# waabox/domain-mcp-server

Hardware: AMD Instinct MI355X
Metric: classes indexed/sec (higher is better)
Workload: dtype n/a (CPU text indexing); 1 GPU; model=synthetic-java-spring-monorepo-2000-classes, global_batch=2000, parallelism=dp1 (one repo per rank), enrichment=none

## Files before the change

native/srcscan/project.cpp:

```cpp
#include <algorithm>
#include <chrono>
#include <dirent.h>
#include <string>
#include <unordered_map>
#include <unordered_set>

#include "srcscan.hpp"

namespace srcscan {

void go_project_files(const std::string& root, int threads, std::string& module, std::vector<FileRec>& files,
                      std::string* go_json);

namespace {

struct Entry {
    std::string name;
    bool is_dir;
};

std::vector<Entry> entries(const std::string& dir) {
    std::vector<std::pair<std::string, bool>> raw;
    std::vector<Entry> out;
    if (!list_dir(dir, raw)) return out;
// ... 41 lines not shown
    w.str_array("deps", f.deps);
    w.key("params");
    w.begin_obj();
    for (auto& kv : f.params) w.str_array(kv.first, kv.second);
    w.end_obj();
    w.key("methods");
    w.begin_arr();
    for (auto& m : f.methods) {
        w.begin_obj();
        w.kv("name", m.name);
        w.kv_int("line", m.line);
        w.kv_opt("httpMethod", m.has_http_method ? &m.http_method : nullptr);
        w.kv_opt("httpPath", m.has_http_path ? &m.http_path : nullptr);
        w.str_array("exceptions", m.exceptions);
        w.end_obj();
    }
    w.end_arr();
    w.end_obj();
}

void scan_java(const std::string& root, const ScanOptions& opt, ScanResult& res) {
    std::vector<FileRec>& files = res.files;
    const std::string src_root = "src/main/java";
    std::string abs_src = join_path(root, src_root);
    if (!dir_exists(abs_src)) return;
    std::vector<std::string> rels;
    auto t = std::chrono::steady_clock::now();
    walk(abs_src, "", [](const std::string& n) { return ends_with(n, ".java"); },
         [](const std::string&) { return false; }, rels);
    res.walk_us = us_since(t);
    t = std::chrono::steady_clock::now();
    files.resize(rels.size());
    std::vector<std::string> sources(rels.size());
    parallel_for(rels.size(), opt.threads, [&](size_t k) {
        FileRec& f = files[k];
        f.rel_path = src_root + "/" + rels[k];
        f.abs_path = join_path(root, f.rel_path);
        f.identifier = dotted(strip_ext(rels[k], ".java"));
        std::string src;
        if (!read_file(f.abs_path, src)) return;
        analyze_java(src, f);
    });
    for (auto& f : files) if (!f.parsed) ++res.skipped;
    res.analyze_us = us_since(t);
    t = std::chrono::steady_clock::now();
    std::unordered_set<std::string> known;
    known.reserve(files.size() * 2);
    for (auto& f : files) known.insert(f.identifier);
    parallel_for(files.size(), opt.threads, [&](size_t k) {
        FileRec& f = files[k];
        std::unordered_set<std::string> seen;
        std::unordered_map<std::string, std::string> import_map;
        for (auto& imp : f.imports) {
            if (imp.is_asterisk) continue;
            std::string fq = imp.imported;
            if (imp.is_static) {
                size_t d = fq.rfind('.');
                fq = (d != std::string::npos && d > 0) ? fq.substr(0, d) : std::string();
            }
            if (fq.empty()) continue;
            size_t d = fq.rfind('.');
            if (d != std::string::npos && d > 0) import_map[fq.substr(d + 1)] = fq;
            if (known.count(fq) && seen.insert(fq).second) f.deps.push_back(fq);
        }
        for (auto& m : f.methods) {
            if (!m.params_eligible || m.param_types.empty()) continue;
            std::vector<std::string> matched;
            for (auto& ty : m.param_types) {
                if (ty.empty()) continue;
                if (known.count(ty)) { matched.push_back(ty); continue; }
                auto it = import_map.find(ty);
                if (it != import_map.end() && known.count(it->second)) { matched.push_back(it->second); continue; }
                if (!f.package_name.empty()) {
                    std::string same = f.package_name + "." + ty;
                    if (known.count(same)) matched.push_back(same);
                }
            }
            if (matched.empty()) continue;
            bool replaced = false;
            for (auto& kv : f.params)
                if (kv.first == m.name) { kv.second = matched; replaced = true; break; }
            if (!replaced) f.params.emplace_back(m.name, matched);
        }
    });
    res.resolve_us = us_since(t);
}

const std::unordered_set<std::string> kTsExcludedDirs = {"node_modules", "dist", ".next", "build",
                                                         "coverage", "__tests__", "__mocks__"};

bool ts_source_file(const std::string& name) {
    if (!(ends_with(name, ".ts") || ends_with(name, ".tsx") || ends_with(name, ".js") || ends_with(name, ".jsx")))
        return false;
    if (contains(name, ".spec.") || contains(name, ".test.")) return false;
    if (ends_with(name, ".d.ts")) return false;
    return true;
}

void scan_ts(const std::string& root, const ScanOptions& opt, std::vector<FileRec>& files, int& skipped,
             FrameworkInfo& fw, std::string& source_root) {
    std::string pkg;
    if (!read_file(join_path(root, "package.json"), pkg)) pkg = "{}";
    fw = detect_framework(pkg);
    if (!opt.framework.empty()) fw.name = opt.framework;
    source_root = dir_exists(join_path(root, fw.source_root)) ? fw.source_root : "src";
    std::string abs_src = join_path(root, source_root);
    std::vector<std::string> rels;
    if (dir_exists(abs_src))
        walk(abs_src, "", ts_source_file, [](const std::string& n) { return kTsExcludedDirs.count(n) > 0; }, rels);
    files.resize(rels.size());
    std::string fw_name = fw.name;
    parallel_for(rels.size(), opt.threads, [&](size_t k) {
        FileRec& f = files[k];
        f.rel_path = source_root + "/" + rels[k];
        f.abs_path = join_path(root, f.rel_path);
        std::string r = rels[k];
        size_t dot = r.rfind('.');
        size_t slash = r.rfind('/');
        if (dot != std::string::npos && dot > 0 && (slash == std::string::npos || dot > slash + 1 || dot > slash))
            r = r.substr(0, dot);
        f.identifier = dotted(r);
        std::string src;
        if (!read_file(f.abs_path, src, opt.max_file_bytes)) return;
        bool jsx = !ends_with(f.rel_path, ".ts");
        analyze_ts(src, f.rel_path, fw_name, jsx, f);
    });
    std::vector<FileRec> kept;
    kept.reserve(files.size());
    for (auto& f : files) {
        if (f.parsed) kept.push_back(std::move(f));
        else ++skipped;
    }
    files.swap(kept);
    std::unordered_set<std::string> known;
    for (auto& f : files) known.insert(f.identifier);
    const std::string abs_root_norm = normalize_path(abs_src);
    auto resolve = [&](const std::string& import_path, const std::string& file_rel) -> std::string {
        std::string dir = file_rel;
        size_t s = dir.rfind('/');
        dir = s == std::string::npos ? std::string() : dir.substr(0, s);
        std::string full = normalize_path(join_path(join_path(root, dir), import_path));
        std::string prefix = abs_root_norm + "/";
        if (!starts_with(full, prefix)) return std::string();
        std::string cand = dotted(full.substr(prefix.size()));
        if (known.count(cand)) return cand;
        std::string idx = cand + ".index";
        if (known.count(idx)) return idx;
        return std::string();
    };
    parallel_for(files.size(), opt.threads, [&](size_t k) {
        FileRec& f = files[k];
        std::unordered_set<std::string> seen;
        std::unordered_map<std::string, std::string> type_map;
        for (auto& imp : f.imports) {
            if (!starts_with(imp.source, ".")) continue;
            std::string r = resolve(imp.source, f.rel_path);
            if (r.empty()) continue;
            if (seen.insert(r).second) f.deps.push_back(r);
            type_map[imp.local] = r;
        }
        for (auto& m : f.methods) {
            std::vector<std::string> matched;
            for (auto& ty : m.param_types) {
                auto it = type_map.find(ty);
                if (it != type_map.end() && known.count(it->second)) matched.push_back(it->second);
            }
            if (matched.empty()) continue;
            bool replaced = false;
            for (auto& kv : f.params)
                if (kv.first == m.name) { kv.second = matched; replaced = true; break; }
            if (!replaced) f.params.emplace_back(m.name, matched);
        }
    });
}

}

std::string detect_language(const std::string& root) {
    if (file_exists(join_path(root, "go.mod"))) return "go";
    if (file_exists(join_path(root, "package.json")) && !file_exists(join_path(root, "pom.xml")) &&
        !file_exists(join_path(root, "build.gradle")) && !file_exists(join_path(root, "build.gradle.kts")))
        return "typescript";
    return "java";
}

ScanResult scan_project(const std::string& root, const ScanOptions& opt) {
    ScanResult r;
    scan_project_into(root, opt, r);
    return r;
}

void scan_project_into(const std::string& root, const ScanOptions& opt, ScanResult& r) {
    auto t0 = std::chrono::steady_clock::now();
    std::string lang = opt.language;
    if (lang == "auto" || lang.empty()) lang = detect_language(root);
    if (lang == "ts" || lang == "js" || lang == "javascript" || lang == "node") lang = "typescript";
    if (lang == "typescript") {
        scan_ts(root, opt, r.files, r.skipped, r.framework, r.source_root);
        r.has_framework = true;
    } else if (lang == "go") {
        go_project_files(root, opt.threads, r.module, r.files, opt.go_doc ? &r.go_json : nullptr);
    } else {
        lang = "java";
        r.source_root = "src/main/java";
        scan_java(root, opt, r);
    }
    r.language = lang;
    r.elapsed_us = std::chrono::duration_cast<std::chrono::microseconds>(std::chrono::steady_clock::now() - t0).count();
}

std::string scan_result_json(const ScanResult& r) {
    JsonWriter w;
    w.begin_obj();
    w.kv("language", r.language);
    w.kv("sourceRoot", r.source_root);
    w.key("framework");
    if (r.has_framework) {
        w.begin_obj();
        w.kv("name", r.framework.name);
        w.kv("sourceRoot", r.framework.source_root);
        w.key("features");
        w.begin_obj();
        for (auto& kv : r.framework.features) w.kv(kv.first, kv.second);
        w.end_obj();
        w.end_obj();
    } else {
        w.value_null();
    }
    if (r.language == "go") w.kv("module", r.module);
    w.key("stats");
    w.begin_obj();
// ... 93 lines not shown
```

native/srcscan/pymodule.cpp:

```cpp
#include <pybind11/pybind11.h>
#include <pybind11/stl.h>
#include <sys/random.h>

#include <cctype>
#include <chrono>
#include <cstring>
#include <deque>
#include <memory>
#include <thread>
#include <unordered_map>
#include <vector>

#include "bulkwriter.hpp"
#include "gitobj.hpp"
#include "graphjson.hpp"
#include "srcscan.hpp"
#include "wire.hpp"

namespace py = pybind11;

namespace {

dbw::Batch to_batch(const std::string& sql, py::handle rows) {
    dbw::Batch b;
    b.sql = sql;
    PyObject* seq = PySequence_Fast(rows.ptr(), "rows must be a sequence");
    if (!seq) throw py::error_already_set();
    py::object keep = py::reinterpret_steal<py::object>(seq);
    const Py_ssize_t n = PySequence_Fast_GET_SIZE(seq);
    if (n == 0) return b;
    PyObject** items = PySequence_Fast_ITEMS(seq);
    PyObject* first = items[0];
    if (!PyTuple_Check(first)) throw py::type_error("rows must be tuples");
    b.ncols = static_cast<int>(PyTuple_GET_SIZE(first));
    b.values.resize(static_cast<size_t>(n) * b.ncols);
    for (Py_ssize_t r = 0; r < n; ++r) {
        PyObject* row = items[r];
        if (!PyTuple_Check(row) || PyTuple_GET_SIZE(row) != b.ncols) throw py::type_error("ragged rows");
        for (int c = 0; c < b.ncols; ++c) {
            PyObject* o = PyTuple_GET_ITEM(row, c);
            dbw::Value& v = b.values[static_cast<size_t>(r) * b.ncols + c];
            if (o == Py_None) {
                v.kind = dbw::Value::Null;
            } else if (PyUnicode_Check(o)) {
                Py_ssize_t len = 0;
                const char* s = PyUnicode_AsUTF8AndSize(o, &len);
                if (!s) throw py::error_already_set();
                v.kind = dbw::Value::Text;
                v.p = s;
                v.n = static_cast<int32_t>(len);
            } else if (PyBool_Check(o) || PyLong_Check(o)) {
                v.kind = dbw::Value::Int;
                v.i = PyLong_AsLongLong(o);
                if (v.i == -1 && PyErr_Occurred()) throw py::error_already_set();
            } else if (PyFloat_Check(o)) {
                v.kind = dbw::Value::Real;
                v.d = PyFloat_AS_DOUBLE(o);
            } else {
                throw py::type_error("unsupported column value type");
            }
        }
    }
    return b;
}

srcscan::ScanResult scan_mounted(py::list files, const std::string& language, int threads,
                                 const std::string& framework, bool go_doc = true) {
    const auto t = std::chrono::steady_clock::now();
    std::vector<py::object> hold;
    hold.reserve(files.size());
    std::vector<std::pair<std::string, std::string_view>> tree;
    tree.reserve(files.size());
    for (auto item : files) {
        auto tup = item.cast<py::tuple>();
        if (tup.size() != 2) throw py::type_error("files: (path, bytes) pairs expected");
        PyObject* content = tup[1].ptr();
        char* data = nullptr;
        Py_ssize_t n = 0;
        if (!PyBytes_Check(content) || PyBytes_AsStringAndSize(content, &data, &n) < 0)
            throw py::type_error("files: content must be bytes");
        tree.emplace_back(tup[0].cast<std::string>(), std::string_view(data, static_cast<size_t>(n)));
        hold.push_back(std::move(tup));
    }
    py::gil_scoped_release release;
    std::string root = srcscan::vfs_mount_views(tree);
    const long long mount_us =
        std::chrono::duration_cast<std::chrono::microseconds>(std::chrono::steady_clock::now() - t).count();
    srcscan::ScanOptions opt;
    opt.language = language;
    opt.threads = threads;
    opt.framework = framework;
    opt.go_doc = go_doc;
    try {
        srcscan::ScanResult r = srcscan::scan_project(root, opt);
        r.mount_us = mount_us;
        srcscan::vfs_unmount(root);
        return r;
    } catch (...) {
        srcscan::vfs_unmount(root);
        throw;
    }
}

py::str pystr(const std::string& s) {
    PyObject* o = PyUnicode_DecodeUTF8(s.data(), static_cast<Py_ssize_t>(s.size()), "replace");
    if (!o) throw py::error_already_set();
    return py::reinterpret_steal<py::str>(o);
}

void json_str_list_ascii(PyObject* seq, std::string& out) {
    static const char* hex = "0123456789abcdef";
    out.push_back('[');
    const Py_ssize_t n = PySequence_Fast_GET_SIZE(seq);
    PyObject** items = PySequence_Fast_ITEMS(seq);
    for (Py_ssize_t i = 0; i < n; ++i) {
        if (i) out.append(", ");
        PyObject* o = items[i];
        if (!PyUnicode_Check(o)) throw py::type_error("exception names must be str");
        out.push_back('"');
        const Py_ssize_t len = PyUnicode_GET_LENGTH(o);
        const int kind = PyUnicode_KIND(o);
        const void* data = PyUnicode_DATA(o);
        for (Py_ssize_t k = 0; k < len; ++k) {
            const Py_UCS4 c = PyUnicode_READ(kind, data, k);
            auto u4 = [&](unsigned v) {
                out.append("\\u");
                for (int sh = 12; sh >= 0; sh -= 4) out.push_back(hex[(v >> sh) & 15]);
            };
            switch (c) {
                case '"': out.append("\\\""); break;
                case '\\': out.append("\\\\"); break;
                case '\n': out.append("\\n"); break;
                case '\r': out.append("\\r"); break;
                case '\t': out.append("\\t"); break;
// ... 156 lines not shown
        PyObject* methods = PyList_New(static_cast<Py_ssize_t>(f.methods.size()));
        if (!methods) throw py::error_already_set();
        for (size_t i = 0; i < f.methods.size(); ++i) {
            const srcscan::MethodRec& m = f.methods[i];
            PyObject* exc = PyTuple_New(static_cast<Py_ssize_t>(m.exceptions.size()));
            if (!exc) throw py::error_already_set();
            for (size_t j = 0; j < m.exceptions.size(); ++j) PyTuple_SET_ITEM(exc, j, shared.get(m.exceptions[j]));
            PyObject* obj = mtype->tp_alloc(mtype, 5);
            if (!obj) throw py::error_already_set();
            PyTuple_SET_ITEM(obj, 0, fresh(m.name));
            PyTuple_SET_ITEM(obj, 1, PyLong_FromLong(m.line));
            PyTuple_SET_ITEM(obj, 2, m.has_http_method ? shared.get(m.http_method) : Py_NewRef(Py_None));
            PyTuple_SET_ITEM(obj, 3, m.has_http_path ? fresh(m.http_path) : Py_NewRef(Py_None));
            PyTuple_SET_ITEM(obj, 4, exc);
            PyList_SET_ITEM(methods, i, obj);
        }
        PyObject* rec = PyTuple_New(8);
        if (!rec) throw py::error_already_set();
        PyTuple_SET_ITEM(rec, 0, fresh(f.rel_path));
        PyTuple_SET_ITEM(rec, 1, fresh(f.identifier));
        PyTuple_SET_ITEM(rec, 2, shared.get(f.class_type));
        PyTuple_SET_ITEM(rec, 3, PyBool_FromLong(f.entry_point));
        PyTuple_SET_ITEM(rec, 4, shared.get(f.package_name));
        PyTuple_SET_ITEM(rec, 5, shared_list(f.deps));
        PyTuple_SET_ITEM(rec, 6, params);
        PyTuple_SET_ITEM(rec, 7, methods);
        PyList_SET_ITEM(files.ptr(), k, rec);
    }
    d["files"] = files;
    d["go"] = r.go_json.empty() ? py::object(py::none()) : py::object(pystr(r.go_json));
    return d;
}

struct Uuid7Gen {
    unsigned long long ms = 0, hi = 0, lo = 0;
    Uuid7Gen() {
        unsigned char seed[10];
        if (getrandom(seed, sizeof(seed), 0) != (ssize_t)sizeof(seed)) throw std::runtime_error("getrandom failed");
        ms = (unsigned long long)std::chrono::duration_cast<std::chrono::milliseconds>(
                 std::chrono::system_clock::now().time_since_epoch())
                 .count();
        hi = ((unsigned long long)(seed[0] & 0x07) << 8) | seed[1];
        for (int j = 2; j < 10; ++j) lo = (lo << 8) | seed[j];
        lo &= 0x1FFFFFFFFFFFFFFFull;
    }
    void next(char* s) {
        static const char* hex = "0123456789abcdef";
        unsigned char b[16];
        for (int j = 0; j < 6; ++j) b[j] = (unsigned char)(ms >> (8 * (5 - j)));
        b[6] = (unsigned char)(0x70 | ((hi >> 8) & 0x0F));
        b[7] = (unsigned char)(hi & 0xFF);
        b[8] = (unsigned char)(0x80 | ((lo >> 56) & 0x3F));
        for (int j = 9; j < 16; ++j) b[j] = (unsigned char)(lo >> (8 * (15 - j)));
        if (++lo >> 62) {
            lo = 0;
            ++hi;
        }
        int k = 0;
        for (int j = 0; j < 16; ++j) {
            if (j == 4 || j == 6 || j == 8 || j == 10) s[k++] = '-';
            s[k++] = hex[b[j] >> 4];
            s[k++] = hex[b[j] & 15];
        }
    }
};

void json_ascii_list(const std::vector<std::string>& v, std::string& out) {
    static const char* hex = "0123456789abcdef";
    auto u4 = [&](unsigned c) {
        out += "\\u";
        for (int sh = 12; sh >= 0; sh -= 4) out += hex[(c >> sh) & 15];
    };
    out = "[";
    for (size_t i = 0; i < v.size(); ++i) {
        if (i) out += ", ";
        out += '"';
        const std::string& s = v[i];
        for (size_t k = 0; k < s.size();) {
            unsigned char c = (unsigned char)s[k];
            unsigned cp = c;
            size_t len = 1;
            if (c >= 0xF0 && k + 3 < s.size() + 0) { cp = ((c & 7u) << 18) | ((s[k + 1] & 63u) << 12) | ((s[k + 2] & 63u) << 6) | (s[k + 3] & 63u); len = 4; }
            else if (c >= 0xE0 && k + 2 < s.size()) { cp = ((c & 15u) << 12) | ((s[k + 1] & 63u) << 6) | (s[k + 2] & 63u); len = 3; }
            else if (c >= 0xC0 && k + 1 < s.size()) { cp = ((c & 31u) << 6) | (s[k + 1] & 63u); len = 2; }
            k += len;
            if (cp == '"') out += "\\\"";
            else if (cp == '\\') out += "\\\\";
            else if (cp == '\n') out += "\\n";
            else if (cp == '\r') out += "\\r";
            else if (cp == '\t') out += "\\t";
            else if (cp == '\b') out += "\\b";
            else if (cp == '\f') out += "\\f";
            else if (cp < 0x20 || (cp >= 0x7f && cp < 0x10000)) u4(cp);
            else if (cp >= 0x10000) {
                cp -= 0x10000;
                u4(0xD800 + (cp >> 10));
                u4(0xDC00 + (cp & 0x3FF));
            } else out += (char)cp;
        }
        out += '"';
    }
    out += "]";
}

struct StaticRowsSpec {
    dbw::BulkWriter* writer = nullptr;
    std::string pid, now, commit, cls_sql, meth_sql;
    bool commit_null = false;
};

struct StaticRowsKeep {
    std::shared_ptr<const srcscan::ScanResult> r;
    StaticRowsSpec spec;
    std::string ids;
    std::vector<size_t> first;
    std::deque<std::string> strings;
};

const std::string& normalize_class_type(const std::string& t) {
    static const std::string kTypes[] = {"CONTROLLER", "SERVICE", "REPOSITORY", "ENTITY", "DTO",
                                         "CONFIGURATION", "LISTENER", "UTILITY", "EXCEPTION", "OTHER"};
    for (const std::string& k : kTypes) {
        if (k.size() != t.size()) continue;
        bool eq = true;
        for (size_t i = 0; i < t.size() && eq; ++i) eq = std::toupper((unsigned char)t[i]) == k[i];
        if (eq) return k;
    }
    return kTypes[9];
}

void emit_static_rows(const std::shared_ptr<StaticRowsKeep>& keep) {
    const srcscan::ScanResult& r = *keep->r;
    const StaticRowsSpec& spec = keep->spec;
    std::unordered_map<std::string_view, size_t> last;
    last.reserve(r.files.size() * 2);
    size_t n_ids = 0;
    for (size_t k = 0; k < r.files.size(); ++k) last[r.files[k].identifier] = k;
    for (size_t k = 0; k < r.files.size(); ++k)
        if (last[r.files[k].identifier] == k) n_ids += 1 + r.files[k].methods.size();
    keep->ids.resize(36 * n_ids);
    keep->first.assign(r.files.size(), std::string::npos);
    Uuid7Gen gen;
    size_t at = 0;
    const int chunk = 256;
    RowBuilder cls(spec.cls_sql, 10), meth(spec.meth_sql, 10);
    int pending = 0;
    auto flush = [&]() {
        cls.b.keep = keep;
        meth.b.keep = keep;
        if (!cls.empty()) spec.writer->put(std::move(cls.b));
        if (!meth.empty()) spec.writer->put(std::move(meth.b));
        cls = RowBuilder(spec.cls_sql, 10);
        meth = RowBuilder(spec.meth_sql, 10);
        pending = 0;
    };
    auto sv = [](RowBuilder& b, const std::string& s) { b.text(s.data(), (Py_ssize_t)s.size()); };
    for (size_t k = 0; k < r.files.size(); ++k) {
        const srcscan::FileRec& f = r.files[k];
        if (last[f.identifier] != k) continue;
        if (pending == chunk) flush();
        ++pending;
        keep->first[k] = at;
        const char* cid = &keep->ids[at];
        gen.next(&keep->ids[at]);
        at += 36;
        const std::string& ident = f.identifier;
        const size_t dot = ident.rfind('.');
        cls.text(cid, 36);
        sv(cls, spec.pid);
        sv(cls, ident);
        if (dot != std::string::npos) cls.text(ident.data() + dot + 1, (Py_ssize_t)(ident.size() - dot - 1));
        else sv(cls, ident);
        if (dot != std::string::npos) cls.text(ident.data(), (Py_ssize_t)dot); else cls.null();
        sv(cls, normalize_class_type(f.class_type));
        cls.null();
        sv(cls, f.rel_path);
        sv(cls, spec.now);
        if (spec.commit_null) cls.null(); else sv(cls, spec.commit);
        for (const srcscan::MethodRec& m : f.methods) {
            gen.next(&keep->ids[at]);
            meth.text(&keep->ids[at], 36);
            at += 36;
            meth.text(cid, 36);
            sv(meth, m.name);
            meth.null();
            meth.text("[]", 2);
            if (m.exceptions.empty()) {
                meth.text("[]", 2);
            } else {
                keep->strings.emplace_back();
                json_ascii_list(m.exceptions, keep->strings.back());
                sv(meth, keep->strings.back());
            }
            if (m.has_http_method) sv(meth, m.http_method); else meth.null();
            if (m.has_http_path) sv(meth, m.http_path); else meth.null();
            meth.integer(m.line);
            sv(meth, spec.now);
        }
    }
    flush();
}

py::tuple phase1_rows(dbw::BulkWriter& writer, py::list order, py::dict units, py::object ids, py::str pid,
                      py::str now, py::handle commit_hash, const std::string& cls_sql, const std::string& meth_sql,
                      const std::string& param_sql, py::handle method_info_cls, int chunk, py::object graph_targets,
                      py::object pre_ids) {
    if (!PyType_Check(method_info_cls.ptr()) ||
        !PyType_IsSubtype((PyTypeObject*)method_info_cls.ptr(), &PyTuple_Type))
        throw py::type_error("method_info_cls must be a tuple subclass");
    auto* mi_type = (PyTypeObject*)method_info_cls.ptr();
    const bool given = !ids.is_none();
    if (given && !PyList_Check(ids.ptr())) throw py::type_error("ids must be a list or None");
    const bool pre = !pre_ids.is_none();
    if (pre && (given || !PyDict_Check(pre_ids.ptr()))) throw py::type_error("pre_ids must be a dict (and ids None)");
    const Py_ssize_t n_ids = given ? PyList_GET_SIZE(ids.ptr()) : 0;
    Py_ssize_t next_id = 0;
    py::list generated;
    Uuid7Gen gen;
    auto nid = [&]() -> PyObject* {
        if (given) {
            if (next_id >= n_ids) throw py::value_error("phase1_rows: ran out of ids");
            return PyList_GET_ITEM(ids.ptr(), next_id++);
        }
        char buf[36];
        gen.next(buf);
        PyObject* o = PyUnicode_FromStringAndSize(buf, 36);
        if (!o || PyList_Append(generated.ptr(), o) < 0) {
            Py_XDECREF(o);
            throw py::error_already_set();
        }
        Py_DECREF(o);
// ... 221 lines not shown
                py::object posn = py::int_(p);
                PyObject* f = PyTuple_Pack(2, posn.ptr(), t);
                if (!f) throw py::error_already_set();
                py::object keep_f = py::reinterpret_steal<py::object>(f);
                py::object link = py::reinterpret_steal<py::object>(make_record(mpl_type, f));
                lks.append(link);
            }
            if (lks.empty()) continue;
            if (!gper) {
                gper = PyDict_GetItemWithError(g_mparams.ptr(), key);
                if (!gper) {
                    if (PyErr_Occurred()) throw py::error_already_set();
                    py::dict fresh;
                    if (PyDict_SetItem(g_mparams.ptr(), key, fresh.ptr()) < 0) throw py::error_already_set();
                    gper = fresh.ptr();
                }
            }
            PyObject* lst = PyDict_GetItemWithError(gper, mname);
            if (!lst) {
                if (PyErr_Occurred()) throw py::error_already_set();
                if (PyDict_SetItem(gper, mname, lks.ptr()) < 0) throw py::error_already_set();
            } else if (PyList_SetSlice(lst, PY_SSIZE_T_MAX, PY_SSIZE_T_MAX, lks.ptr()) < 0) {
                throw py::error_already_set();
            }
        }
    }
    if (!par.empty()) writer.put(std::move(par.b));
    return py::make_tuple(n_cls, n_meth, n_par, class_ids, class_types, method_infos, methods_by_ident, links,
                          generated);
}

}

py::dict objects_and_rows(std::shared_ptr<const srcscan::ScanResult> shared, py::handle method_cls, py::object rows) {
    std::shared_ptr<StaticRowsKeep> keep;
    std::thread emitter;
    std::atomic<long long> emit_us{0};
    if (!rows.is_none() && shared->language != "go") {
        py::tuple rt = rows.cast<py::tuple>();
        if (rt.size() != 6) throw py::value_error("rows must have 6 items");
        keep = std::make_shared<StaticRowsKeep>();
        keep->r = shared;
        StaticRowsSpec& spec = keep->spec;
        spec.writer = &rt[0].cast<dbw::BulkWriter&>();
        spec.pid = rt[1].cast<std::string>();
        spec.now = rt[2].cast<std::string>();
        spec.commit_null = rt[3].is_none();
        if (!spec.commit_null) spec.commit = rt[3].cast<std::string>();
        spec.cls_sql = rt[4].cast<std::string>();
        spec.meth_sql = rt[5].cast<std::string>();
        emitter = std::thread([keep, &emit_us] {
            const auto t = std::chrono::steady_clock::now();
            emit_static_rows(keep);
            emit_us = std::chrono::duration_cast<std::chrono::microseconds>(
                          std::chrono::steady_clock::now() - t).count();
        });
    }
    py::dict d;
    try {
        const auto t = std::chrono::steady_clock::now();
        d = scan_result_objects(*shared, method_cls);
        py::dict(d["stats"])["phaseUs"].cast<py::dict>()["objects"] =
            std::chrono::duration_cast<std::chrono::microseconds>(std::chrono::steady_clock::now() - t)
                .count();
    } catch (...) {
        if (emitter.joinable()) {
            py::gil_scoped_release release;
            emitter.join();
        }
        throw;
    }
    if (emitter.joinable()) {
        {
            py::gil_scoped_release release;
            emitter.join();
        }
        py::dict(d["stats"])["phaseUs"].cast<py::dict>()["rows"] = emit_us.load();
        py::dict row_ids;
        for (size_t k = 0; k < shared->files.size(); ++k) {
            const size_t at = keep->first[k];
            if (at == std::string::npos) continue;
            const size_t nm = shared->files[k].methods.size();
            py::list mids(nm);
            for (size_t j = 0; j < nm; ++j) mids[j] = py::str(&keep->ids[at + 36 * (j + 1)], 36);
            row_ids[pystr(shared->files[k].identifier)] = py::make_tuple(py::str(&keep->ids[at], 36), mids);
        }
        d["rowIds"] = row_ids;
    }
    keep.reset();
    std::thread([](std::shared_ptr<const srcscan::ScanResult>) {}, std::move(shared)).detach();
    return d;
}

PYBIND11_MODULE(_srcscan, m) {
    m.doc() = "Native Java / TypeScript / Go source front-ends for dmcp";
    m.def(
        "scan_project",
        [](const std::string& root, const std::string& language, int threads, const std::string& framework) {
            std::string out;
            {
                py::gil_scoped_release release;
                srcscan::ScanOptions opt;
                opt.language = language;
                opt.threads = threads;
                opt.framework = framework;
                out = srcscan::scan_project_json(root, opt);
            }
            return py::bytes(out);
        },
        py::arg("root"), py::arg("language") = "auto", py::arg("threads") = 0, py::arg("framework") = "");
    m.def(
        "scan_sources",
        [](py::list files, const std::string& language, int threads, const std::string& framework) {
            std::vector<std::pair<std::string, std::string>> tree;
            tree.reserve(files.size());
            for (auto item : files) {
                auto tup = item.cast<py::tuple>();
                tree.emplace_back(tup[0].cast<std::string>(), tup[1].cast<std::string>());
            }
            std::string out;
            {
                py::gil_scoped_release release;
                std::string root = srcscan::vfs_mount(std::move(tree));
                srcscan::ScanOptions opt;
                opt.language = language;
                opt.threads = threads;
                opt.framework = framework;
                try {
                    out = srcscan::scan_project_json(root, opt);
                } catch (...) {
                    srcscan::vfs_unmount(root);
                    throw;
                }
                srcscan::vfs_unmount(root);
            }
            return py::bytes(out);
        },
        py::arg("files"), py::arg("language") = "auto", py::arg("threads") = 0, py::arg("framework") = "");
    m.def(
        "scan_sources_objects",
        [](py::list files, const std::string& language, int threads, const std::string& framework,
           py::handle method_cls, py::object rows, bool go_doc) {
            auto r = std::make_unique<srcscan::ScanResult>(scan_mounted(files, language, threads, framework,
                                                                        go_doc));
            return objects_and_rows(std::shared_ptr<const srcscan::ScanResult>(std::move(r)), method_cls, rows);
        },
        py::arg("files"), py::arg("language"), py::arg("threads"), py::arg("framework"), py::arg("method_cls"),
        py::arg("rows") = py::none(), py::arg("go_doc") = true,
        "scan_sources as Python objects (files as tuples, methods as method_cls) -- no JSON round trip; "
        "with rows, the class / method rows are written first (ids in 'rowIds'); go_doc=False: no "
        "go-analyzer package document (Go)");
    m.def(
        "result_objects",
        [](py::bytes blob, py::handle method_cls, py::object rows) {
            auto r = std::make_unique<srcscan::ScanResult>();
            std::string err;
            bool ok;
            {
                char* data = nullptr;
                Py_ssize_t n = 0;
                if (PyBytes_AsStringAndSize(blob.ptr(), &data, &n) < 0) throw py::error_already_set();
                py::gil_scoped_release release;
                ok = srcscan::decode_result(std::string_view(data, static_cast<size_t>(n)), *r, err);
            }
            if (!ok) throw py::value_error("scan result: " + err);
            return objects_and_rows(std::shared_ptr<const srcscan::ScanResult>(std::move(r)), method_cls, rows);
        },
        py::arg("blob"), py::arg("method_cls"), py::arg("rows") = py::none(),
        "the binary ScanResult of `srcscan serve` as scan_sources_objects returns it (untrusted bytes: every "
        "length checked)");
    m.def(
        "encode_scan",
        [](py::list files, const std::string& language, int threads, const std::string& framework, bool go_doc) {
            srcscan::ScanResult r = scan_mounted(files, language, threads, framework, go_doc);
            std::string out;
            {
                py::gil_scoped_release release;
                out = srcscan::encode_result(r, true);
            }
            return py::bytes(out);
        },
        py::arg("files"), py::arg("language"), py::arg("threads"), py::arg("framework"), py::arg("go_doc") = true);
    m.def(
        "scan_file",
// ... 213 lines not shown
```

native/srcscan/srcscan.hpp:

```cpp
#pragma once

#include <string>
#include <vector>

#include "common.hpp"

namespace srcscan {

struct MethodRec {
    std::string name;
    int line = 0;
    bool has_http_method = false, has_http_path = false;
    std::string http_method, http_path;
    std::vector<std::string> exceptions;
    std::vector<std::string> param_types;
    bool is_ctor = false;
    bool params_eligible = true;
};

struct ImportRec {
    std::string imported;
    std::string local;
    std::string source;
    bool is_static = false;
    bool is_asterisk = false;
};

struct FileRec {
    std::string abs_path;
    std::string rel_path;
    std::string identifier;
    std::string class_type = "OTHER";
    bool entry_point = false;
    bool parsed = false;
    std::string package_name;
    std::vector<MethodRec> methods;
    std::vector<ImportRec> imports;
    std::vector<std::string> deps;
    std::vector<std::pair<std::string, std::vector<std::string>>> params;
};

void analyze_java(std::string_view src, FileRec& out);

void analyze_ts(std::string_view src, const std::string& rel_path, const std::string& framework,
                bool jsx, FileRec& out);

struct FrameworkInfo {
    std::string name = "unknown";
    std::string source_root = "src";
    std::vector<std::pair<std::string, std::string>> features;
};
FrameworkInfo detect_framework(std::string_view package_json);

struct GoProject;
std::string analyze_go_project_json(const std::string& root, int threads);

struct ScanOptions {
    std::string language = "auto";
    int threads = 0;
    std::string framework;
    size_t max_file_bytes = 5u * 1024u * 1024u;
    bool go_doc = true;
};

struct ScanResult {
    std::string language;
    std::string source_root = ".";
    bool has_framework = false;
    FrameworkInfo framework;
    std::string module;
    std::string go_json;
    std::vector<FileRec> files;
    int skipped = 0;
    long long elapsed_us = 0;
    long long walk_us = 0, analyze_us = 0, resolve_us = 0, mount_us = 0;
};

ScanResult scan_project(const std::string& root, const ScanOptions& opt);
void scan_project_into(const std::string& root, const ScanOptions& opt, ScanResult& r);

std::string scan_project_json(const std::string& root, const ScanOptions& opt);
std::string scan_result_json(const ScanResult& r);

std::string scan_file_json(const std::string& path, const std::string& language,
                           const std::string& rel_path, const std::string& framework);
std::string analyze_source_json(const std::string& content, const std::string& language, const std::string& file_path,
                                const std::string& framework);

std::string detect_language(const std::string& root);

}
```

Measured before the change: 51090 classes/s.

## Stream DB row emission concurrently with per-file source analysis

Adds a FileSink hook to the Java/TS scanners and a RowStreamer thread that builds and queues class/method rows as files finish parsing, instead of emitting all rows after the scan completes. File names are computed up front so duplicate identifiers can be resolved in order as results arrive. This overlaps row construction with analysis and resolution, at the cost of mutex/condvar traffic per file and extra copies of the file records for TS when files are skipped. It is enabled by default unless DMCP_STREAM_ROWS=0.

```diff
diff --git a/native/srcscan/project.cpp b/native/srcscan/project.cpp
--- a/native/srcscan/project.cpp
+++ b/native/srcscan/project.cpp
@@ -97,15 +97,25 @@
     t = std::chrono::steady_clock::now();
     files.resize(rels.size());
     std::vector<std::string> sources(rels.size());
-    parallel_for(rels.size(), opt.threads, [&](size_t k) {
+    auto name_file = [&](size_t k) {
         FileRec& f = files[k];
         f.rel_path = src_root + "/" + rels[k];
         f.abs_path = join_path(root, f.rel_path);
         f.identifier = dotted(strip_ext(rels[k], ".java"));
+    };
+    FileSink* sink = opt.sink;
+    if (sink) {
+        for (size_t k = 0; k < rels.size(); ++k) name_file(k);
+        sink->begin(files, false);
+    }
+    parallel_for(rels.size(), opt.threads, [&](size_t k) {
+        FileRec& f = files[k];
+        if (!sink) name_file(k);
         std::string src;
-        if (!read_file(f.abs_path, src)) return;
-        analyze_java(src, f);
+        if (read_file(f.abs_path, src)) analyze_java(src, f);
+        if (sink) sink->file_done(k);
     });
+    if (sink) sink->analyzed();
     for (auto& f : files) if (!f.parsed) ++res.skipped;
     res.analyze_us = us_since(t);
     t = std::chrono::steady_clock::now();
@@ -162,8 +172,11 @@
     return true;
 }
 
-void scan_ts(const std::string& root, const ScanOptions& opt, std::vector<FileRec>& files, int& skipped,
-             FrameworkInfo& fw, std::string& source_root) {
+void scan_ts(const std::string& root, const ScanOptions& opt, ScanResult& res) {
+    std::vector<FileRec>& files = res.files;
+    int& skipped = res.skipped;
+    FrameworkInfo& fw = res.framework;
+    std::string& source_root = res.source_root;
     std::string pkg;
     if (!read_file(join_path(root, "package.json"), pkg)) pkg = "{}";
     fw = detect_framework(pkg);
@@ -175,7 +188,7 @@
         walk(abs_src, "", ts_source_file, [](const std::string& n) { return kTsExcludedDirs.count(n) > 0; }, rels);
     files.resize(rels.size());
     std::string fw_name = fw.name;
-    parallel_for(rels.size(), opt.threads, [&](size_t k) {
+    auto name_file = [&](size_t k) {
         FileRec& f = files[k];
         f.rel_path = source_root + "/" + rels[k];
         f.abs_path = join_path(root, f.rel_path);
@@ -185,18 +198,35 @@
         if (dot != std::string::npos && dot > 0 && (slash == std::string::npos || dot > slash + 1 || dot > slash))
             r = r.substr(0, dot);
         f.identifier = dotted(r);
+    };
+    FileSink* sink = opt.sink;
+    if (sink) {
+        for (size_t k = 0; k < rels.size(); ++k) name_file(k);
+        sink->begin(files, true);
+    }
+    parallel_for(rels.size(), opt.threads, [&](size_t k) {
+        FileRec& f = files[k];
+        if (!sink) name_file(k);
         std::string src;
-        if (!read_file(f.abs_path, src, opt.max_file_bytes)) return;
-        bool jsx = !ends_with(f.rel_path, ".ts");
-        analyze_ts(src, f.rel_path, fw_name, jsx, f);
+        if (read_file(f.abs_path, src, opt.max_file_bytes)) {
+            bool jsx = !ends_with(f.rel_path, ".ts");
+            analyze_ts(src, f.rel_path, fw_name, jsx, f);
+        }
+        if (sink) sink->file_done(k);
     });
-    std::vector<FileRec> kept;
-    kept.reserve(files.size());
-    for (auto& f : files) {
-        if (f.parsed) kept.push_back(std::move(f));
-        else ++skipped;
-    }
-    files.swap(kept);
+    if (sink) sink->analyzed();
+    for (auto& f : files) if (!f.parsed) ++skipped;
+    if (skipped) {
+        std::vector<FileRec> kept;
+        kept.reserve(files.size() - skipped);
+        if (sink) {
+            for (auto& f : files) if (f.parsed) kept.push_back(f);
+            res.sink_files.swap(files);
+        } else {
+            for (auto& f : files) if (f.parsed) kept.push_back(std::move(f));
+        }
+        files.swap(kept);
+    }
     std::unordered_set<std::string> known;
     for (auto& f : files) known.insert(f.identifier);
     const std::string abs_root_norm = normalize_path(abs_src);
@@ -261,7 +291,7 @@
     if (lang == "auto" || lang.empty()) lang = detect_language(root);
     if (lang == "ts" || lang == "js" || lang == "javascript" || lang == "node") lang = "typescript";
     if (lang == "typescript") {
-        scan_ts(root, opt, r.files, r.skipped, r.framework, r.source_root);
+        scan_ts(root, opt, r);
         r.has_framework = true;
     } else if (lang == "go") {
         go_project_files(root, opt.threads, r.module, r.files, opt.go_doc ? &r.go_json : nullptr);
diff --git a/native/srcscan/pymodule.cpp b/native/srcscan/pymodule.cpp
--- a/native/srcscan/pymodule.cpp
+++ b/native/srcscan/pymodule.cpp
@@ -14,12 +14,15 @@
 #include "bulkwriter.hpp"
 #include "gitobj.hpp"
 #include "graphjson.hpp"
+#include "rowstream.hpp"
 #include "srcscan.hpp"
 #include "wire.hpp"
 
 namespace py = pybind11;
 
 namespace {
+
+using namespace rowstream;
 
 dbw::Batch to_batch(const std::string& sql, py::handle rows) {
     dbw::Batch b;
@@ -64,8 +67,8 @@
     return b;
 }
 
-srcscan::ScanResult scan_mounted(py::list files, const std::string& language, int threads,
-                                 const std::string& framework, bool go_doc = true) {
+void scan_mounted_into(py::list files, const std::string& language, int threads, const std::string& framework,
+                       bool go_doc, srcscan::ScanResult& r, srcscan::FileSink* sink = nullptr) {
     const auto t = std::chrono::steady_clock::now();
     std::vector<py::object> hold;
     hold.reserve(files.size());
@@ -91,15 +94,22 @@
     opt.threads = threads;
     opt.framework = framework;
     opt.go_doc = go_doc;
+    opt.sink = sink;
     try {
-        srcscan::ScanResult r = srcscan::scan_project(root, opt);
+        srcscan::scan_project_into(root, opt, r);
         r.mount_us = mount_us;
         srcscan::vfs_unmount(root);
-        return r;
     } catch (...) {
         srcscan::vfs_unmount(root);
         throw;
     }
+}
+
+srcscan::ScanResult scan_mounted(py::list files, const std::string& language, int threads,
+                                 const std::string& framework, bool go_doc = true) {
+    srcscan::ScanResult r;
+    scan_mounted_into(files, language, threads, framework, go_doc, r);
+    return r;
 }
 
 py::str pystr(const std::string& s) {
@@ -322,83 +332,6 @@
     return d;
 }
 
-struct Uuid7Gen {
-    unsigned long long ms = 0, hi = 0, lo = 0;
-    Uuid7Gen() {
-        unsigned char seed[10];
-        if (getrandom(seed, sizeof(seed), 0) != (ssize_t)sizeof(seed)) throw std::runtime_error("getrandom failed");
-        ms = (unsigned long long)std::chrono::duration_cast<std::chrono::milliseconds>(
-                 std::chrono::system_clock::now().time_since_epoch())
-                 .count();
-        hi = ((unsigned long long)(seed[0] & 0x07) << 8) | seed[1];
-        for (int j = 2; j < 10; ++j) lo = (lo << 8) | seed[j];
-        lo &= 0x1FFFFFFFFFFFFFFFull;
-    }
-    void next(char* s) {
-        static const char* hex = "0123456789abcdef";
-        unsigned char b[16];
-        for (int j = 0; j < 6; ++j) b[j] = (unsigned char)(ms >> (8 * (5 - j)));
-        b[6] = (unsigned char)(0x70 | ((hi >> 8) & 0x0F));
-        b[7] = (unsigned char)(hi & 0xFF);
-        b[8] = (unsigned char)(0x80 | ((lo >> 56) & 0x3F));
-        for (int j = 9; j < 16; ++j) b[j] = (unsigned char)(lo >> (8 * (15 - j)));
-        if (++lo >> 62) {
-            lo = 0;
-            ++hi;
-        }
-        int k = 0;
-        for (int j = 0; j < 16; ++j) {
-            if (j == 4 || j == 6 || j == 8 || j == 10) s[k++] = '-';
-            s[k++] = hex[b[j] >> 4];
-            s[k++] = hex[b[j] & 15];
-        }
-    }
-};
-
-void json_ascii_list(const std::vector<std::string>& v, std::string& out) {
-    static const char* hex = "0123456789abcdef";
-    auto u4 = [&](unsigned c) {
-        out += "\\u";
-        for (int sh = 12; sh >= 0; sh -= 4) out += hex[(c >> sh) & 15];
-    };
-    out = "[";
-    for (size_t i = 0; i < v.size(); ++i) {
-        if (i) out += ", ";
-        out += '"';
-        const std::string& s = v[i];
-        for (size_t k = 0; k < s.size();) {
-            unsigned char c = (unsigned char)s[k];
-            unsigned cp = c;
-            size_t len = 1;
-            if (c >= 0xF0 && k + 3 < s.size() + 0) { cp = ((c & 7u) << 18) | ((s[k + 1] & 63u) << 12) | ((s[k + 2] & 63u) << 6) | (s[k + 3] & 63u); len = 4; }
-            else if (c >= 0xE0 && k + 2 < s.size()) { cp = ((c & 15u) << 12) | ((s[k + 1] & 63u) << 6) | (s[k + 2] & 63u); len = 3; }
-            else if (c >= 0xC0 && k + 1 < s.size()) { cp = ((c & 31u) << 6) | (s[k + 1] & 63u); len = 2; }
-            k += len;
-            if (cp == '"') out += "\\\"";
-            else if (cp == '\\') out += "\\\\";
-            else if (cp == '\n') out += "\\n";
-            else if (cp == '\r') out += "\\r";
-            else if (cp == '\t') out += "\\t";
-            else if (cp == '\b') out += "\\b";
-            else if (cp == '\f') out += "\\f";
-            else if (cp < 0x20 || (cp >= 0x7f && cp < 0x10000)) u4(cp);
-            else if (cp >= 0x10000) {
-                cp -= 0x10000;
-                u4(0xD800 + (cp >> 10));
-                u4(0xDC00 + (cp & 0x3FF));
-            } else out += (char)cp;
-        }
-        out += '"';
-    }
-    out += "]";
-}
-
-struct StaticRowsSpec {
-    dbw::BulkWriter* writer = nullptr;
-    std::string pid, now, commit, cls_sql, meth_sql;
-    bool commit_null = false;
-};
-
 struct StaticRowsKeep {
     std::shared_ptr<const srcscan::ScanResult> r;
     StaticRowsSpec spec;
@@ -406,18 +339,6 @@
     std::vector<size_t> first;
     std::deque<std::string> strings;
 };
-
-const std::string& normalize_class_type(const std::string& t) {
-    static const std::string kTypes[] = {"CONTROLLER", "SERVICE", "REPOSITORY", "ENTITY", "DTO",
-                                         "CONFIGURATION", "LISTENER", "UTILITY", "EXCEPTION", "OTHER"};
-    for (const std::string& k : kTypes) {
-        if (k.size() != t.size()) continue;
-        bool eq = true;
-        for (size_t i = 0; i < t.size() && eq; ++i) eq = std::toupper((unsigned char)t[i]) == k[i];
-        if (eq) return k;
-    }
-    return kTypes[9];
-}
 
 void emit_static_rows(const std::shared_ptr<StaticRowsKeep>& keep) {
     const srcscan::ScanResult& r = *keep->r;
@@ -444,49 +365,19 @@
         meth = RowBuilder(spec.meth_sql, 10);
         pending = 0;
     };
-    auto sv = [](RowBuilder& b, const std::string& s) { b.text(s.data(), (Py_ssize_t)s.size()); };
+    auto next_id = [&]() {
+        char* p = &keep->ids[at];
+        gen.next(p);
+        at += 36;
+        return (const char*)p;
+    };
     for (size_t k = 0; k < r.files.size(); ++k) {
         const srcscan::FileRec& f = r.files[k];
         if (last[f.identifier] != k) continue;
         if (pending == chunk) flush();
         ++pending;
         keep->first[k] = at;
-        const char* cid = &keep->ids[at];
-        gen.next(&keep->ids[at]);
-        at += 36;
-        const std::string& ident = f.identifier;
-        const size_t dot = ident.rfind('.');
-        cls.text(cid, 36);
-        sv(cls, spec.pid);
-        sv(cls, ident);
-        if (dot != std::string::npos) cls.text(ident.data() + dot + 1, (Py_ssize_t)(ident.size() - dot - 1));
-        else sv(cls, ident);
-        if (dot != std::string::npos) cls.text(ident.data(), (Py_ssize_t)dot); else cls.null();
-        sv(cls, normalize_class_type(f.class_type));
-        cls.null();
-        sv(cls, f.rel_path);
-        sv(cls, spec.now);
-        if (spec.commit_null) cls.null(); else sv(cls, spec.commit);
-        for (const srcscan::MethodRec& m : f.methods) {
-            gen.next(&keep->ids[at]);
-            meth.text(&keep->ids[at], 36);
-            at += 36;
-            meth.text(cid, 36);
-            sv(meth, m.name);
-            meth.null();
-            meth.text("[]", 2);
-            if (m.exceptions.empty()) {
-                meth.text("[]", 2);
-            } else {
-                keep->strings.emplace_back();
-                json_ascii_list(m.exceptions, keep->strings.back());
-                sv(meth, keep->strings.back());
-            }
-            if (m.has_http_method) sv(meth, m.http_method); else meth.null();
-            if (m.has_http_path) sv(meth, m.http_path); else meth.null();
-            meth.integer(m.line);
-            sv(meth, spec.now);
-        }
+        add_file_rows(spec, f, cls, meth, keep->strings, next_id);
     }
     flush();
 }
@@ -774,23 +665,28 @@
 
 }
 
+StaticRowsSpec rows_spec(const py::object& rows) {
+    py::tuple rt = rows.cast<py::tuple>();
+    if (rt.size() != 6) throw py::value_error("rows must have 6 items");
+    StaticRowsSpec spec;
+    spec.writer = &rt[0].cast<dbw::BulkWriter&>();
+    spec.pid = rt[1].cast<std::string>();
+    spec.now = rt[2].cast<std::string>();
+    spec.commit_null = rt[3].is_none();
+    if (!spec.commit_null) spec.commit = rt[3].cast<std::string>();
+    spec.cls_sql = rt[4].cast<std::string>();
+    spec.meth_sql = rt[5].cast<std::string>();
+    return spec;
+}
+
 py::dict objects_and_rows(std::shared_ptr<const srcscan::ScanResult> shared, py::handle method_cls, py::object rows) {
     std::shared_ptr<StaticRowsKeep> keep;
     std::thread emitter;
     std::atomic<long long> emit_us{0};
     if (!rows.is_none() && shared->language != "go") {
-        py::tuple rt = rows.cast<py::tuple>();
-        if (rt.size() != 6) throw py::value_error("rows must have 6 items");
         keep = std::make_shared<StaticRowsKeep>();
         keep->r = shared;
-        StaticRowsSpec& spec = keep->spec;
-        spec.writer = &rt[0].cast<dbw::BulkWriter&>();
-        spec.pid = rt[1].cast<std::string>();
-        spec.now = rt[2].cast<std::string>();
-        spec.commit_null = rt[3].is_none();
-        if (!spec.commit_null) spec.commit = rt[3].cast<std::string>();
-        spec.cls_sql = rt[4].cast<std::string>();
-        spec.meth_sql = rt[5].cast<std::string>();
+        keep->spec = rows_spec(rows);
         emitter = std::thread([keep, &emit_us] {
             const auto t = std::chrono::steady_clock::now();
             emit_static_rows(keep);
@@ -830,6 +726,52 @@
         d["rowIds"] = row_ids;
     }
     keep.reset();
+    std::thread([](std::shared_ptr<const srcscan::ScanResult>) {}, std::move(shared)).detach();
+    return d;
+}
+
+py::dict scan_objects_streamed(py::list files, const std::string& language, int threads,
+                               const std::string& framework, py::handle method_cls, py::object rows, bool go_doc) {
+    auto result = std::make_shared<srcscan::ScanResult>();
+    std::shared_ptr<const srcscan::ScanResult> shared = result;
+    RowStreamer streamer(shared, rows_spec(rows));
+    auto stop = [&]() {
+        streamer.cancel();
+        py::gil_scoped_release release;
+        try {
+            streamer.join();
+        } catch (...) {
+        }
+    };
+    py::dict d;
+    try {
+        scan_mounted_into(files, language, threads, framework, go_doc, *result, &streamer);
+        streamer.analyzed();
+        const auto t = std::chrono::steady_clock::now();
+        d = scan_result_objects(*shared, method_cls);
+        py::dict(d["stats"])["phaseUs"].cast<py::dict>()["objects"] =
+            std::chrono::duration_cast<std::chrono::microseconds>(std::chrono::steady_clock::now() - t).count();
+    } catch (...) {
+        stop();
+        throw;
+    }
+    {
+        py::gil_scoped_release release;
+        streamer.join();
+    }
+    if (shared->language != "go") {
+        py::dict(d["stats"])["phaseUs"].cast<py::dict>()["rows"] = streamer.busy_us();
+        const RowStreamer::State& st = streamer.state();
+        py::dict row_ids;
+        for (const RowStreamer::Emitted& e : st.emitted) {
+            const size_t nm = e.file->methods.size();
+            py::list mids(nm);
+            for (size_t j = 0; j < nm; ++j) mids[j] = py::str(st.ids.at(e.first_id + 1 + j), 36);
+            row_ids[pystr(e.file->identifier)] = py::make_tuple(py::str(st.ids.at(e.first_id), 36), mids);
+        }
+        d["rowIds"] = row_ids;
+    }
+    result.reset();
     std::thread([](std::shared_ptr<const srcscan::ScanResult>) {}, std::move(shared)).detach();
     return d;
 }
@@ -883,6 +825,8 @@
         "scan_sources_objects",
         [](py::list files, const std::string& language, int threads, const std::string& framework,
            py::handle method_cls, py::object rows, bool go_doc) {
+            if (!rows.is_none() && stream_rows_enabled())
+                return scan_objects_streamed(files, language, threads, framework, method_cls, rows, go_doc);
             auto r = std::make_unique<srcscan::ScanResult>(scan_mounted(files, language, threads, framework,
                                                                         go_doc));
             return objects_and_rows(std::shared_ptr<const srcscan::ScanResult>(std::move(r)), method_cls, rows);
@@ -892,6 +836,15 @@
         "scan_sources as Python objects (files as tuples, methods as method_cls) -- no JSON round trip; "
         "with rows, the class / method rows are written first (ids in 'rowIds'); go_doc=False: no "
         "go-analyzer package document (Go)");
+    m.def(
+        "stream_rows",
+        [](py::object on) {
+            if (!on.is_none()) set_stream_rows(on.cast<bool>());
+            return stream_rows_enabled();
+        },
+        py::arg("on") = py::none(),
+        "whether scan_sources_objects(rows=...) emits its rows while the scan runs (DMCP_STREAM_ROWS, read "
+        "once); with an argument: sets it (in-process A/B runs)");
     m.def(
         "result_objects",
         [](py::bytes blob, py::handle method_cls, py::object rows) {
diff --git a/native/srcscan/rowstream.hpp b/native/srcscan/rowstream.hpp
--- /dev/null
+++ b/native/srcscan/rowstream.hpp
@@ -0,0 +1,358 @@
+#pragma once
+
+#include <sys/random.h>
+
+#include <atomic>
+#include <cctype>
+#include <chrono>
+#include <condition_variable>
+#include <cstdlib>
+#include <deque>
+#include <exception>
+#include <memory>
+#include <mutex>
+#include <stdexcept>
+#include <string>
+#include <string_view>
+#include <thread>
+#include <unordered_map>
+#include <vector>
+
+#include "bulkwriter.hpp"
+#include "srcscan.hpp"
+
+namespace rowstream {
+
+struct Uuid7Gen {
+    unsigned long long ms = 0, hi = 0, lo = 0;
+    Uuid7Gen() {
+        unsigned char seed[10];
+        if (getrandom(seed, sizeof(seed), 0) != (ssize_t)sizeof(seed)) throw std::runtime_error("getrandom failed");
+        ms = (unsigned long long)std::chrono::duration_cast<std::chrono::milliseconds>(
+                 std::chrono::system_clock::now().time_since_epoch())
+                 .count();
+        hi = ((unsigned long long)(seed[0] & 0x07) << 8) | seed[1];
+        for (int j = 2; j < 10; ++j) lo = (lo << 8) | seed[j];
+        lo &= 0x1FFFFFFFFFFFFFFFull;
+    }
+    void next(char* s) {
+        static const char* hex = "0123456789abcdef";
+        unsigned char b[16];
+        for (int j = 0; j < 6; ++j) b[j] = (unsigned char)(ms >> (8 * (5 - j)));
+        b[6] = (unsigned char)(0x70 | ((hi >> 8) & 0x0F));
+        b[7] = (unsigned char)(hi & 0xFF);
+        b[8] = (unsigned char)(0x80 | ((lo >> 56) & 0x3F));
+        for (int j = 9; j < 16; ++j) b[j] = (unsigned char)(lo >> (8 * (15 - j)));
+        if (++lo >> 62) {
+            lo = 0;
+            ++hi;
+        }
+        int k = 0;
+        for (int j = 0; j < 16; ++j) {
+            if (j == 4 || j == 6 || j == 8 || j == 10) s[k++] = '-';
+            s[k++] = hex[b[j] >> 4];
+            s[k++] = hex[b[j] & 15];
+        }
+    }
+};
+
+inline void json_ascii_list(const std::vector<std::string>& v, std::string& out) {
+    static const char* hex = "0123456789abcdef";
+    auto u4 = [&](unsigned c) {
+        out += "\\u";
+        for (int sh = 12; sh >= 0; sh -= 4) out += hex[(c >> sh) & 15];
+    };
+    out = "[";
+    for (size_t i = 0; i < v.size(); ++i) {
+        if (i) out += ", ";
+        out += '"';
+        const std::string& s = v[i];
+        for (size_t k = 0; k < s.size();) {
+            unsigned char c = (unsigned char)s[k];
+            unsigned cp = c;
+            size_t len = 1;
+            if (c >= 0xF0 && k + 3 < s.size() + 0) { cp = ((c & 7u) << 18) | ((s[k + 1] & 63u) << 12) | ((s[k + 2] & 63u) << 6) | (s[k + 3] & 63u); len = 4; }
+            else if (c >= 0xE0 && k + 2 < s.size()) { cp = ((c & 15u) << 12) | ((s[k + 1] & 63u) << 6) | (s[k + 2] & 63u); len = 3; }
+            else if (c >= 0xC0 && k + 1 < s.size()) { cp = ((c & 31u) << 6) | (s[k + 1] & 63u); len = 2; }
+            k += len;
+            if (cp == '"') out += "\\\"";
+            else if (cp == '\\') out += "\\\\";
+            else if (cp == '\n') out += "\\n";
+            else if (cp == '\r') out += "\\r";
+            else if (cp == '\t') out += "\\t";
+            else if (cp == '\b') out += "\\b";
+            else if (cp == '\f') out += "\\f";
+            else if (cp < 0x20 || (cp >= 0x7f && cp < 0x10000)) u4(cp);
+            else if (cp >= 0x10000) {
+                cp -= 0x10000;
+                u4(0xD800 + (cp >> 10));
+                u4(0xDC00 + (cp & 0x3FF));
+            } else out += (char)cp;
+        }
+        out += '"';
+    }
+    out += "]";
+}
+
+
+struct StaticRowsSpec {
+    dbw::BulkWriter* writer = nullptr;
+    std::string pid, now, commit, cls_sql, meth_sql;
+    bool commit_null = false;
+};
+
+
+inline const std::string& normalize_class_type(const std::string& t) {
+    static const std::string kTypes[] = {"CONTROLLER", "SERVICE", "REPOSITORY", "ENTITY", "DTO",
+                                         "CONFIGURATION", "LISTENER", "UTILITY", "EXCEPTION", "OTHER"};
+    for (const std::string& k : kTypes) {
+        if (k.size() != t.size()) continue;
+        bool eq = true;
+        for (size_t i = 0; i < t.size() && eq; ++i) eq = std::toupper((unsigned char)t[i]) == k[i];
+        if (eq) return k;
+    }
+    return kTypes[9];
+}
+
+template <class Rows, class NextId>
+void add_file_rows(const StaticRowsSpec& spec, const srcscan::FileRec& f, Rows& cls, Rows& meth,
+                   std::deque<std::string>& strings, NextId&& next_id) {
+    auto sv = [](Rows& b, const std::string& s) { b.text(s.data(), (long)s.size()); };
+    const char* cid = next_id();
+    const std::string& ident = f.identifier;
+    const size_t dot = ident.rfind('.');
+    cls.text(cid, 36);
+    sv(cls, spec.pid);
+    sv(cls, ident);
+    if (dot != std::string::npos) cls.text(ident.data() + dot + 1, (long)(ident.size() - dot - 1));
+    else sv(cls, ident);
+    if (dot != std::string::npos) cls.text(ident.data(), (long)dot); else cls.null();
+    sv(cls, normalize_class_type(f.class_type));
+    cls.null();
+    sv(cls, f.rel_path);
+    sv(cls, spec.now);
+    if (spec.commit_null) cls.null(); else sv(cls, spec.commit);
+    for (const srcscan::MethodRec& m : f.methods) {
+        meth.text(next_id(), 36);
+        meth.text(cid, 36);
+        sv(meth, m.name);
+        meth.null();
+        meth.text("[]", 2);
+        if (m.exceptions.empty()) {
+            meth.text("[]", 2);
+        } else {
+            strings.emplace_back();
+            json_ascii_list(m.exceptions, strings.back());
+            sv(meth, strings.back());
+        }
+        if (m.has_http_method) sv(meth, m.http_method); else meth.null();
+        if (m.has_http_path) sv(meth, m.http_path); else meth.null();
+        meth.integer(m.line);
+        sv(meth, spec.now);
+    }
+}
+
+struct PlainRows {
+    dbw::Batch b;
+    PlainRows(const std::string& sql, int ncols) {
+        b.sql = sql;
+        b.ncols = ncols;
+    }
+    void null() { b.values.emplace_back(); }
+    void text(const char* p, long n) {
+        dbw::Value v;
+        v.kind = dbw::Value::Text;
+        v.p = p;
+        v.n = static_cast<int32_t>(n);
+        b.values.push_back(v);
+    }
+    void integer(long long i) {
+        dbw::Value v;
+        v.kind = dbw::Value::Int;
+        v.i = i;
+        b.values.push_back(v);
+    }
+    bool empty() const { return b.values.empty(); }
+};
+
+class IdPool {
+  public:
+    char* next() {
+        if (n_ % kPer == 0 && n_ / kPer == blocks_.size()) blocks_.emplace_back(new char[36 * kPer]);
+        char* p = blocks_[n_ / kPer].get() + 36 * (n_ % kPer);
+        ++n_;
+        return p;
+    }
+    const char* at(size_t i) const { return blocks_[i / kPer].get() + 36 * (i % kPer); }
+    size_t size() const { return n_; }
+
+  private:
+    static constexpr size_t kPer = 4096;
+    std::vector<std::unique_ptr<char[]>> blocks_;
+    size_t n_ = 0;
+};
+
+inline std::atomic<int>& stream_rows_flag() {
+    static std::atomic<int> flag{[] {
+        const char* e = std::getenv("DMCP_STREAM_ROWS");
+        return (e && e[0] == '0' && e[1] == '\0') ? 0 : 1;
+    }()};
+    return flag;
+}
+inline bool stream_rows_enabled() { return stream_rows_flag().load(std::memory_order_relaxed) != 0; }
+inline void set_stream_rows(bool on) { stream_rows_flag().store(on ? 1 : 0, std::memory_order_relaxed); }
+
+class RowStreamer final : public srcscan::FileSink {
+  public:
+    struct Emitted {
+        const srcscan::FileRec* file;
+        size_t first_id;
+    };
+    struct State {
+        std::shared_ptr<const srcscan::ScanResult> result;
+        StaticRowsSpec spec;
+        IdPool ids;
+        std::deque<std::string> strings;
+        std::vector<Emitted> emitted;
+    };
+
+    RowStreamer(std::shared_ptr<const srcscan::ScanResult> result, StaticRowsSpec spec)
+        : state_(std::make_shared<State>()) {
+        state_->result = std::move(result);
+        state_->spec = std::move(spec);
+        thread_ = std::thread([this] { run(); });
+    }
+    ~RowStreamer() override {
+        cancel();
+        if (thread_.joinable()) thread_.join();
+    }
+    RowStreamer(const RowStreamer&) = delete;
+    RowStreamer& operator=(const RowStreamer&) = delete;
+
+    void begin(const std::vector<srcscan::FileRec>& files, bool drop_unparsed) override {
+        std::vector<size_t> next_same(files.size(), kNone);
+        std::unordered_map<std::string_view, size_t> later;
+        later.reserve(files.size() * 2);
+        for (size_t k = files.size(); k-- > 0;) {
+            auto ins = later.emplace(files[k].identifier, k);
+            if (!ins.second) {
+                next_same[k] = ins.first->second;
+                ins.first->second = k;
+            }
+        }
+        std::lock_guard<std::mutex> lk(mu_);
+        files_ = &files;
+        drop_unparsed_ = drop_unparsed;
+        next_same_ = std::move(next_same);
+    }
+    void file_done(size_t k) override {
+        std::lock_guard<std::mutex> lk(mu_);
+        const bool wake = done_.empty();
+        done_.push_back(k);
+        if (wake) cv_.notify_one();
+    }
+    void analyzed() override {
+        std::lock_guard<std::mutex> lk(mu_);
+        analyzed_ = true;
+        cv_.notify_one();
+    }
+    void cancel() {
+        std::lock_guard<std::mutex> lk(mu_);
+        cancelled_ = true;
+        cv_.notify_one();
+    }
+    void join() {
+        if (thread_.joinable()) thread_.join();
+        if (error_) {
+            std::exception_ptr e = error_;
+            error_ = nullptr;
+            std::rethrow_exception(e);
+        }
+    }
+    long long busy_us() const { return busy_us_; }
+    const State& state() const { return *state_; }
+
+  private:
+    void run() {
+        try {
+            emit_loop();
+        } catch (...) {
+            error_ = std::current_exception();
+        }
+    }
+    void emit_loop() {
+        State& st = *state_;
+        const StaticRowsSpec& spec = st.spec;
+        Uuid7Gen gen;
+        const int chunk = 256;
+        PlainRows cls(spec.cls_sql, 10), meth(spec.meth_sql, 10);
+        int pending = 0;
+        auto flush = [&]() {
+            cls.b.keep = state_;
+            meth.b.keep = state_;
+            if (!cls.empty()) spec.writer->put(std::move(cls.b));
+            if (!meth.empty()) spec.writer->put(std::move(meth.b));
+            cls = PlainRows(spec.cls_sql, 10);
+            meth = PlainRows(spec.meth_sql, 10);
+            pending = 0;
+        };
+        auto next_id = [&]() {
+            char* p = st.ids.next();
+            gen.next(p);
+            return (const char*)p;
+        };
+        auto emit = [&](const srcscan::FileRec& f) {
+            if (pending == chunk) flush();
+            ++pending;
+            st.emitted.push_back({&f, st.ids.size()});
+            add_file_rows(spec, f, cls, meth, st.strings, next_id);
+        };
+        std::vector<size_t> batch;
+        std::vector<uint8_t> done;
+        size_t cursor = 0;
+        for (;;) {
+            bool fin;
+            {
+                std::unique_lock<std::mutex> lk(mu_);
+                cv_.wait(lk, [&] { return !done_.empty() || analyzed_ || cancelled_; });
+                if (cancelled_) return;
+                batch.clear();
+                batch.swap(done_);
+                fin = analyzed_;
+            }
+            if (!files_) return;
+            const auto t = std::chrono::steady_clock::now();
+            const std::vector<srcscan::FileRec>& files = *files_;
+            if (done.size() != files.size()) done.assign(files.size(), 0);
+            for (size_t k : batch) done[k] = 1;
+            auto eligible = [&](size_t k) { return !drop_unparsed_ || files[k].parsed; };
+            for (; cursor < files.size() && done[cursor]; ++cursor) {
+                bool wins = eligible(cursor), decided = true;
+                for (size_t j = next_same_[cursor]; j != kNone && decided; j = next_same_[j]) {
+                    if (!done[j]) decided = false;
+                    else if (eligible(j)) wins = false;
+                }
+                if (!decided) break;
+                if (wins) emit(files[cursor]);
+            }
+            if (fin) flush();
+            busy_us_ += std::chrono::duration_cast<std::chrono::microseconds>(std::chrono::steady_clock::now() - t)
+                            .count();
+            if (fin) return;
+        }
+    }
+
+    std::shared_ptr<State> state_;
+    std::mutex mu_;
+    std::condition_variable cv_;
+    std::vector<size_t> done_;
+    const std::vector<srcscan::FileRec>* files_ = nullptr;
+    static constexpr size_t kNone = static_cast<size_t>(-1);
+    std::vector<size_t> next_same_;
+    bool drop_unparsed_ = false, analyzed_ = false, cancelled_ = false;
+    std::thread thread_;
+    std::exception_ptr error_;
+    long long busy_us_ = 0;
+};
+
+}
diff --git a/native/srcscan/srcscan.hpp b/native/srcscan/srcscan.hpp
--- a/native/srcscan/srcscan.hpp
+++ b/native/srcscan/srcscan.hpp
@@ -55,12 +55,20 @@
 struct GoProject;
 std::string analyze_go_project_json(const std::string& root, int threads);
 
+struct FileSink {
+    virtual ~FileSink() = default;
+    virtual void begin(const std::vector<FileRec>& files, bool drop_unparsed) = 0;
+    virtual void file_done(size_t k) = 0;
+    virtual void analyzed() = 0;
+};
+
 struct ScanOptions {
     std::string language = "auto";
     int threads = 0;
     std::string framework;
     size_t max_file_bytes = 5u * 1024u * 1024u;
     bool go_doc = true;
+    FileSink* sink = nullptr;
 };
 
 struct ScanResult {
@@ -71,6 +79,7 @@
     std::string module;
     std::string go_json;
     std::vector<FileRec> files;
+    std::vector<FileRec> sink_files;
     int skipped = 0;
     long long elapsed_us = 0;
     long long walk_us = 0, analyze_us = 0, resolve_us = 0, mount_us = 0;
```

After: 48280 classes/s. -5.5%, worse.
